# antonilo/unsupervised_detection

Hardware: NVIDIA H100
Metric: frame-pairs/sec adversarial train step 256x448 (higher is better)
Workload: dtype bf16

## Files before the change

### include/cis_b200.h

```cpp
#ifndef CIS_B200_H_
#define CIS_B200_H_
#include <stdint.h>
#include <stddef.h>

#ifdef __cplusplus
extern "C" {
#endif

typedef void* cis_stream_t;

enum { CIS_OK = 0, CIS_ERR_BAD_ARG = 1, CIS_ERR_UNSUPPORTED = 2, CIS_ERR_CUDA = 3 };
enum { CIS_ACT_NONE = 0, CIS_ACT_ELU = 1, CIS_ACT_LEAKY = 2 };
enum { CIS_MAX_TAPS = 49, CIS_MAX_SRC = 4 };

typedef struct {
  const void* ptr;
  int32_t pitch;
  int32_t c_off;
  int32_t chunks;
  int32_t n_mod;
} CisSrc;

typedef struct {
  int32_t N, H, W;
// ... 58 lines not shown
  int32_t Cout;
  int32_t K_pad;
  int32_t splits;
  int32_t tma;
  int32_t nh;
  int32_t nwg;
} CisWgrad;

const char* cis_last_error(void);
int cis_version(void);
uint32_t cis_crc32c(uint32_t crc, const void* data, size_t n);
int cis_host_resize_bilinear_legacy(const float* src, int32_t H, int32_t W, int32_t C, float* dst, int32_t OH, int32_t OW);
int cis_host_bgr8_to_rgb_resized(const unsigned char* bgr, int32_t H, int32_t W, float* dst, int32_t OH, int32_t OW);

int cis_conv_igemm(const CisConv* d, cis_stream_t stream);
int cis_set_persist_mode(int mode);
int cis_conv_wgrad(const CisWgrad* d, cis_stream_t stream);

int cis_pack_weights(const float* w, const int32_t* kmap, int32_t K_pad, int32_t rows, int32_t cout, int32_t sn, const int32_t* nmap,
                     void* wp, cis_stream_t stream);
int cis_pack_weights_tiled(const float* w, const int32_t* kmap, int32_t cin8, int32_t ntaps, int32_t n_tiles, int32_t BN, int32_t cout,
                           int32_t sn, const int32_t* nmap, void* out, int32_t thin, cis_stream_t stream);
int cis_unpack_wgrad(const float* dwp, const int32_t* kmap, int32_t K_pad, int32_t cout, int32_t nsplit, float* dw, const float* colpart,
                     int32_t nblocks, int32_t nch, float* db, int32_t layout, cis_stream_t stream);
int cis_bn_fold(const float* w, const float* bias, const float* gamma, const float* beta, int64_t nw, int32_t cout, float* w_eff,
                float* b_eff, cis_stream_t stream);
int cis_bn_chain(const float* w, const float* bias, const float* gamma, float* dw_eff_to_dw, const float* db_eff, int64_t nw,
                 int32_t cout, float* dbias, float* dgamma, float* dbeta, cis_stream_t stream);

enum { CIS_JOB_PACK = 0, CIS_JOB_PACK_TILED = 1, CIS_JOB_UNPACK = 2, CIS_JOB_BN_FOLD = 3, CIS_JOB_BN_CHAIN = 4 };
// ... 124 lines not shown
```

### unsupervised_detection_b200/_lib.py

```python
import ctypes as C
import os

_HERE = os.path.dirname(os.path.abspath(__file__))
LIB_PATH = os.path.join(_HERE, os.environ.get('CIS_LIB_NAME', 'libcis_b200.so'))

MAX_TAPS, MAX_SRC = 49, 4
ACT_NONE, ACT_ELU, ACT_LEAKY = 0, 1, 2
RESIZE_BILINEAR, RESIZE_NEAREST = 0, 1


class CisSrc(C.Structure):
    _fields_ = [('ptr', C.c_void_p), ('pitch', C.c_int32), ('c_off', C.c_int32), ('chunks', C.c_int32), ('n_mod', C.c_int32)]


class CisParamJob(C.Structure):
    _fields_ = [('kind', C.c_int32), ('i', C.c_int32 * 8), ('n', C.c_int64), ('p', C.c_void_p * 8)]


JOB_PACK, JOB_PACK_TILED, JOB_UNPACK, JOB_BN_FOLD, JOB_BN_CHAIN = range(5)


class CisSub(C.Structure):
    _fields_ = [('tap0', C.c_int32), ('ntaps', C.c_int32), ('hoy', C.c_int32), ('hox', C.c_int32), ('OH', C.c_int32), ('OW', C.c_int32),
                ('oa', C.c_int32), ('ob', C.c_int32), ('wpack', C.c_void_p)]
# ... 81 lines not shown
    'cis_cast_bf16_to_f32': [_p, _i64, _i32, _i32, _i32, _p],
    'cis_cast_bf16_to_f32_scaled': [_p, _i64, _i32, _i32, _i32, _f32, _p],
    'cis_charbonnier_bwd': [_p, _p, _p, _i32, _i64, _i32, _i32, _f32, _p, _p, _p, _p],
    'cis_dense_image_warp_bwd': [_p, _i32, _i32, _p, _f32, _i32, _i32, _i32, _i32, _p, _p, _p, _p],
    'cis_cost_volume_bwd': [_p, _i32, _i32, _p, _i32, _i32, _p, _i32, _i32, _i32, _i32, _p, _p, _p],
    'cis_resize_f32_bwd_to_bf16_scaled': [_p, _i32, _i32, _i32, _i32, _i32, _i32, _p, _i32, _f32],
    'cis_warp_costvol_bwd': [_p, _i32, _i32, _p, _i32, _i32, _p, _f32, _i32, _i32, _i32, _i32, _p, _i32, _i32, _p, _i32, _i32, _p, _i32, _i32,
                             _p, _i32, _i32, _i32, _p, _p, _p],
    'cis_parity_split_bf16': [_p, _i32, _i32, _i32, _i32, _i32, _i32, _p, _i32],
    'cis_warp_costvol_r': [_p, _i32, _i32, _p, _i32, _i32, _p, _f32, _i32, _i32, _i32, _i32, _p, _i32, _i32, _i32],
    'cis_cost_volume_bwd_r': [_p, _i32, _i32, _p, _i32, _i32, _p, _i32, _i32, _i32, _i32, _p, _p, _p, _i32],
    'cis_warp_costvol_bwd_r': [_p, _i32, _i32, _p, _i32, _i32, _p, _f32, _i32, _i32, _i32, _i32, _p, _i32, _i32, _p, _i32, _i32, _p, _i32, _i32,
                               _p, _i32, _i32, _i32, _p, _p, _p, _i32],
}
EXPORTS = sorted(list(_PROTOS) + ['cis_last_error', 'cis_version', 'cis_set_persist_mode', 'cis_crc32c', 'cis_host_resize_bilinear_legacy',
                                  'cis_host_bgr8_to_rgb_resized'])

_lib = None


def load():
    global _lib
    if _lib is None:
        if not os.path.exists(LIB_PATH):
            raise RuntimeError('libcis_b200.so not built: run `python -c "import __graft_entry__ as g; g.build()"` '
                               '(no CPU fallback exists for the product path)')
        lib = C.CDLL(LIB_PATH)
        lib.cis_last_error.restype = C.c_char_p
        lib.cis_version.restype = C.c_int
        lib.cis_set_persist_mode.argtypes = [C.c_int]
        lib.cis_set_persist_mode.restype = C.c_int
        lib.cis_crc32c.argtypes = [C.c_uint32, C.c_void_p, C.c_size_t]
        lib.cis_crc32c.restype = C.c_uint32
        lib.cis_host_resize_bilinear_legacy.argtypes = [C.c_void_p, C.c_int32, C.c_int32, C.c_int32, C.c_void_p, C.c_int32, C.c_int32]
        lib.cis_host_resize_bilinear_legacy.restype = C.c_int
        lib.cis_host_bgr8_to_rgb_resized.argtypes = [C.c_void_p, C.c_int32, C.c_int32, C.c_void_p, C.c_int32, C.c_int32]
        lib.cis_host_bgr8_to_rgb_resized.restype = C.c_int
        for name, args in _PROTOS.items():
            fn = getattr(lib, name)
            fn.argtypes = list(args) + [C.c_void_p]
            fn.restype = C.c_int
        _lib = lib
    return _lib


def check(rc, what=''):
    if rc != 0:
        raise RuntimeError('libcis_b200 %s failed (code %d): %s' % (what, rc, load().cis_last_error().decode()))


def call(name, *args):
    check(getattr(load(), name)(*args), name)
# ... 1 lines not shown
```

### unsupervised_detection_b200/csrc/conv_igemm.cu

```cuda
#include "ptx.cuh"
#include "../../include/cis_b200.h"
#include "common.cuh"
#include <cuda.h>
#include <stdlib.h>
#include <string.h>


namespace cis {

#ifdef CIS_TRACE
__device__ unsigned long long* g_trace = nullptr;
__device__ int g_trace_cap = 0;
#define CIS_TRACE_AT(slot)                                                                                         \
  do {                                                                                                             \
    if (g_trace && blockIdx.x == 0 && blockIdx.y == 0 && blockIdx.z == 0 && (slot) < g_trace_cap) g_trace[(slot)] = clock64(); \
  } while (0)
#else
#define CIS_TRACE_AT(slot) ((void)0)
#endif

static constexpr int kBM = 128;
static constexpr int kBK = 64;
static constexpr int kAStage = kBM * 128;
static constexpr int kThreads = 256;
// ... 471 lines not shown
        const int t = g / p.OW;
        const int oh = t % p.OH;
        const int n = t / p.OH;
        return (size_t)(n * p.DH + oh * p.osh + p.oa) * p.DW + ow * p.osw + p.ob;
      });
    }
    cluster_sync_all();
  }
  if (tid == 0) CIS_TRACE_AT(3);
}


static constexpr int kHaloMaxBStages = 8;
struct HaloMaps {
  CUtensorMap m[CIS_MAX_SRC * 4];
};

template <int NK, int MT, int BN, int MTM>
__device__ __forceinline__ void halo_issue_stage(float (&acc)[MTM][BN], const uint32_t hlo, uint32_t blo, const uint32_t* s_aoff, const int gt,
                                                 const uint32_t ahi, const uint32_t bhi, const uint32_t a_mstep, const uint32_t a_half,
                                                 const uint32_t bstep, const bool first) {
  uint32_t off0 = s_aoff[0], off1 = gt > 1 ? s_aoff[1] : 0u;
  int tt = 0;
#pragma unroll 1
  do {
    const uint32_t off2 = tt + 2 < gt ? s_aoff[tt + 2] : 0u;
    const uint32_t alo = hlo + off0;
    const uint32_t acc0 = (uint32_t)(!(first && tt == 0));
    wg_fence();
#pragma unroll
    for (int m = 0; m < MT; ++m) {
// ... 21 lines not shown
                                               const uint32_t a_half, const uint32_t bstep, const bool first) {
  static_assert(MTM >= 1 && MTM <= 4, "1..4 stacked tiles");
  if (MT == 1) halo_issue_nk<1>(nk16, acc, hlo, blo, s_aoff, gt, ahi, bhi, a_mstep, a_half, bstep, first);
  else if constexpr (MTM >= 2) {
    if (MT == 2) halo_issue_nk<2>(nk16, acc, hlo, blo, s_aoff, gt, ahi, bhi, a_mstep, a_half, bstep, first);
    else if constexpr (MTM >= 3) {
      if (MT == 3) halo_issue_nk<3>(nk16, acc, hlo, blo, s_aoff, gt, ahi, bhi, a_mstep, a_half, bstep, first);
      else if constexpr (MTM >= 4) halo_issue_nk<4>(nk16, acc, hlo, blo, s_aoff, gt, ahi, bhi, a_mstep, a_half, bstep, first);
    }
  }
  wg_wait<0>();
}

__host__ __device__ __forceinline__ int thin_plane_bytes(int HP) { return (HP * 16 + 127) & ~127; }
__host__ __device__ __forceinline__ int halo_nsteps(int thin, int ntaps) { return thin == 8 ? (ntaps + 1) / 2 : ntaps; }
__device__ __forceinline__ uint32_t halo_step_off(const CisConv& p, const int t0, const int nt, const int s, const int Wh, const uint32_t plane16) {
  if (!p.thin) return (uint32_t)((p.dh[t0 + s] * Wh + p.dw[t0 + s]) * 8);
  const int ta = p.thin == 8 ? 2 * s : s;
  const uint32_t o0 = (uint32_t)(p.dh[t0 + ta] * Wh + p.dw[t0 + ta]);
  if (p.thin == 16) return o0 | (plane16 << 16);
  const uint32_t o1 = ta + 1 < nt ? (uint32_t)(p.dh[t0 + ta + 1] * Wh + p.dw[t0 + ta + 1]) : o0;
  return o0 | ((o1 - o0) << 16);
}

template <int BN, int NWG>
__global__ void __launch_bounds__(HaloCfg<BN, NWG>::kThreads, 1) conv_halo_kernel(const __grid_constant__ CisConv p, const int halo_stage_bytes, const int BS, const int NHS,
                                                        const __grid_constant__ HaloMaps maps, const int use_tma, const int G) {
  using Cfg = HaloCfg<BN, NWG>;
  constexpr int kBStage = BN * 128;
  constexpr int kHMmaWarp_ = Cfg::kMmaWarp, kHThreads_ = Cfg::kThreads;
  extern __shared__ uint8_t smem_raw[];
  __shared__ uint64_t bars[2 * 2 + 2 * kHaloMaxBStages + 1];
  __shared__ uint32_t s_aoff[CIS_MAX_TAPS];
  __shared__ SrcS s_src[CIS_MAX_SRC];

  const int tid = threadIdx.x, warp = tid >> 5, lane = tid & 31;
  const int MT = p.MT, MTC = NWG * MT, d = p.dil;
  const int nph = p.nph > 1 ? p.nph : 1;
  const int Wh = 8 + p.ex, Hh = 16 * MTC + p.ey, HP = Wh * Hh;
  const int thin = p.thin;
  const uint32_t wstep = thin ? BN * 32 : kBStage;
  const uint32_t stage_bytes = (uint32_t)G * wstep;
  const uint32_t tile_base = (smem_u32(smem_raw) + 1023u) & ~1023u;
  const uint32_t h_base = tile_base;
  const uint32_t b_base = tile_base + NHS * halo_stage_bytes;
  int* pixtab = reinterpret_cast<int*>(smem_raw + (b_base + BS * stage_bytes - smem_u32(smem_raw)));
  const uint32_t bar_hfull = smem_u32(&bars[0]), bar_hempty = smem_u32(&bars[2]);
  const uint32_t bar_bfull = smem_u32(&bars[4]), bar_bempty = smem_u32(&bars[4 + kHaloMaxBStages]);
  const uint32_t bar_accum = smem_u32(&bars[4 + 2 * kHaloMaxBStages]);

  const bool grouped = p.nsub > 1;
  const int tap0 = grouped ? p.sub[blockIdx.z].tap0 : 0, ntaps = grouped ? p.sub[blockIdx.z].ntaps : p.ntaps;
  const int nst = halo_nsteps(thin, ntaps);
  const int hoy = grouped ? p.sub[blockIdx.z].hoy : p.hoy, hox = grouped ? p.sub[blockIdx.z].hox : p.hox;
  const int OHs = grouped ? p.sub[blockIdx.z].OH : p.OH, OWs = grouped ? p.sub[blockIdx.z].OW : p.OW;
// ... 44 lines not shown
    }
    mbar_init(bar_accum, 128 * NWG);
    fence_mbar_init();
  }
  if (use_tma && tid < p.nsrc) tma_prefetch_desc(&maps.m[tid]);
  pdl_wait();
  if (tid < BN) s_bias[tid] = p.bias ? p.bias[ny * BN + tid] : 0.f;
  __syncthreads();
  if (tid == 0) CIS_TRACE_AT(0);

  if (warp < kHMmaWarp_) {
   if (warp < 4) {
    if (use_tma) {
      if (tid == 0) {
        int hcount = 0;
        for (int vc = 0; vc < nchunks * nph; ++vc) {
          const int cc = vc / nph, ph = vc - cc * nph;
          if (nph > 1 && p.ph_tap[ph + 1] == p.ph_tap[ph]) continue;
          const int hs = hcount % NHS;
          mbar_wait(bar_hempty + 8 * hs, (uint32_t)(((hcount / NHS) & 1) ^ 1));
          ++hcount;
          int c = (cc_lo + cc) * 8, si = 0;
          while (si < p.nsrc - 1 && c >= s_src[si].chunks) {
            c -= s_src[si].chunks;
            ++si;
          }
          const int nmod = s_src[si].n_mod;
          if (thin) {
            const int npl = thin / 8, pb16 = thin_plane_bytes(HP);
            mbar_expect_tx(bar_hfull + 8 * hs, (uint32_t)(npl * HP * 16));
            for (int q = 0; q < npl; ++q) {
              int cq = q, sq = 0;
              while (sq < p.nsrc - 1 && cq >= s_src[sq].chunks) {
                cq -= s_src[sq].chunks;
                ++sq;
              }
              const int nm = s_src[sq].n_mod;
              tma_load_4d(h_base + hs * halo_stage_bytes + q * pb16, &maps.m[sq], bar_hfull + 8 * hs, cq * 8, tx * 8 + hox, ty * 16 * MTC + hoy,
                          nm ? (n % nm) : n);
            }
            continue;
          }
          mbar_expect_tx(bar_hfull + 8 * hs, (uint32_t)(HP * 128));
          tma_load_4d(h_base + hs * halo_stage_bytes, &maps.m[si * nph + ph], bar_hfull + 8 * hs, c * 8, pb + d * (tx * 8 + hox),
                      pa + d * (ty * 16 * MTC + hoy), nmod ? (n % nmod) : n);
        }
      }
      __syncwarp();
    } else if (warp != 2) {
      const int hid = warp == 3 ? tid - 32 : tid;
      const int j = hid & 7, pl = hid >> 3;
      for (int cc = 0; cc < nchunks; ++cc) {
        const int hs = cc % NHS;
        mbar_wait(bar_hempty + 8 * hs, (uint32_t)(((cc / NHS) & 1) ^ 1));
        const int rem = m_chunks - (cc_lo + cc) * 8;
// ... 31 lines not shown
          cp_async_wait<1>();
          fence_proxy_async();
          mbar_arrive(bar_hfull + 8 * ((cc - 1) % NHS));
        }
      }
      if (NHS > 1) {
        cp_async_wait<0>();
        fence_proxy_async();
        mbar_arrive(bar_hfull + 8 * ((nchunks - 1) % NHS));
      }
    }
    if (tid == 64) {
      const uint8_t* wt = reinterpret_cast<const uint8_t*>(wpack) + ((size_t)ny * nchunks_all + cc_lo) * nst * wstep;
      int bs = 0;
      uint32_t bph = 1;
      for (int vc = 0; vc < nchunks * nph; ++vc) {
        const int cc = vc / nph, ph = vc - cc * nph;
        const int tlo = nph > 1 ? p.ph_tap[ph] : 0, thi = nph > 1 ? p.ph_tap[ph + 1] : nst;
        for (int t0 = tlo; t0 < thi; t0 += G) {
          const uint32_t bytes = (uint32_t)min(G, thi - t0) * wstep;
          mbar_wait(bar_bempty + 8 * bs, bph);
          mbar_expect_tx(bar_bfull + 8 * bs, bytes);
          bulk_g2s(b_base + bs * stage_bytes, wt + (size_t)(cc * nst + t0) * wstep, bytes, bar_bfull + 8 * bs);
          if (++bs == BS) {
            bs = 0;
            bph ^= 1u;
          }
        }
      }
    }
    __syncwarp();
   }

  } else {
    const int wg = NWG > 1 ? (warp - kHMmaWarp_) >> 2 : 0;
    const int wtid = tid - (kHMmaWarp_ + 4 * wg) * 32;
    constexpr int MTM = Cfg::kMaxMT;
    float acc[MTM][BN];
    const uint32_t pix = thin ? 16u : 128u;
    const uint32_t ahi = thin ? desc_hi_ns((uint32_t)Wh * pix) : desc_hi((uint32_t)Wh * pix), bhi = thin ? desc_hi_ns(256) : desc_hi(1024);
    const uint32_t a_mstep = (16u * Wh * pix) >> 4;
    const uint32_t a_half = (8u * Wh * pix) >> 4;
    const uint32_t a_wg = (uint32_t)(wg * MT) * a_mstep;
    int bs = 0, hs = 0, it = 0;
    uint32_t bph = 0, hph = 0;
    bool any = false;
    for (int vc = 0; vc < nchunks * nph; ++vc) {
      const int cc = vc / nph, ph = vc - cc * nph;
      const int tlo = nph > 1 ? p.ph_tap[ph] : 0, thi = nph > 1 ? p.ph_tap[ph + 1] : nst;
      if (thi == tlo) continue;
      const int rem = m_chunks - (cc_lo + cc) * 8;
      const int nk16 = rem >= 8 ? 4 : (rem + 1) / 2;
      mbar_wait(bar_hfull + 8 * hs, hph);
      if (vc == 0 && wtid == 0 && wg == 0) CIS_TRACE_AT(1);
      const uint32_t hlo = desc_lo(h_base + hs * halo_stage_bytes, thin ? 0 : 16) + a_wg;
      for (int t0 = tlo; t0 < thi; t0 += G, ++it) {
        const int gt = min(G, thi - t0);
        mbar_wait(bar_bfull + 8 * bs, bph);
        if (wtid == 0 && wg == 0) CIS_TRACE_AT(8 + 2 * it);
        const uint32_t blo = desc_lo(b_base + bs * stage_bytes, thin ? 128 : 16);
        halo_issue_any<BN, MTM>(nk16, acc, hlo, blo, s_aoff + t0, gt, MT, ahi, bhi, a_mstep, a_half, wstep >> 4, !any);
        if (wtid == 0) {
          mbar_arrive(bar_bempty + 8 * bs);
          if (t0 + G >= thi) mbar_arrive(bar_hempty + 8 * hs);
          if (wg == 0) CIS_TRACE_AT(9 + 2 * it);
        }
        any = true;
        if (++bs == BS) {
          bs = 0;
          bph ^= 1u;
        }
      }
      if (++hs == NHS) {
        hs = 0;
        hph ^= 1u;
// ... 193 lines not shown
        int z, tx, ty, n;
        decode(w, z, tx, ty, n);
        const int hox = grouped ? p.sub[z].hox : p.hox, hoy = grouped ? p.sub[z].hoy : p.hoy;
        for (int cc = 0; cc < nchunks; ++cc) {
          mbar_wait(bar_hempty + 8 * hs, hph);
          int c = cc * 8, si = 0;
          while (si < p.nsrc - 1 && c >= p.src[si].chunks) {
            c -= p.src[si].chunks;
            ++si;
          }
          int nmod = p.src[0].n_mod;
          if (si == 1) nmod = p.src[1].n_mod;
          if (si == 2) nmod = p.src[2].n_mod;
          if (si == 3) nmod = p.src[3].n_mod;
          if (thin) {
            const int npl = thin / 8, pb16 = thin_plane_bytes(HP);
            mbar_expect_tx(bar_hfull + 8 * hs, (uint32_t)(npl * HP * 16));
            for (int q = 0; q < npl; ++q) {
              int cq = q, sq = 0;
              while (sq < p.nsrc - 1 && cq >= p.src[sq].chunks) {
                cq -= p.src[sq].chunks;
                ++sq;
              }
              const int nm = p.src[sq].n_mod;
              tma_load_4d(h_base + hs * halo_stage_bytes + q * pb16, &maps.m[sq], bar_hfull + 8 * hs, cq * 8, tx * 8 + hox, ty * 16 * MT + hoy,
                          nm ? (n % nm) : n);
            }
          } else {
            mbar_expect_tx(bar_hfull + 8 * hs, (uint32_t)(HP * 128));
            tma_load_4d(h_base + hs * halo_stage_bytes, &maps.m[si], bar_hfull + 8 * hs, c * 8, tx * 8 + hox, ty * 16 * MT + hoy,
                        nmod ? (n % nmod) : n);
          }
          if (++hs == NHS) {
            hs = 0;
            hph ^= 1u;
          }
        }
      }
    }
  } else if (warp == 13) {
    if (lane == 0) {
      const uint8_t* wt = reinterpret_cast<const uint8_t*>(p.wpack);
      const int nst = s_sbase[1];
      if (ws) {
        if ((int)blockIdx.x < total) {
          mbar_expect_tx(bar_bfull, (uint32_t)(nchunks * s_sbase[nsb] * wstep));
          for (int z = 0; z < nsb; ++z) {
            const uint8_t* wz = grouped ? reinterpret_cast<const uint8_t*>(p.sub[z].wpack) : wt;
            const int per = nchunks * (s_sbase[z + 1] - s_sbase[z]);
            for (int it = 0; it < per; it += 8) {
              const int nt = min(8, per - it);
              bulk_g2s(b_base + (s_sbase[z] + it) * wstep, wz + (size_t)it * wstep, (uint32_t)(nt * wstep), bar_bfull);
            }
          }
        }
      } else {
        int bs = 0;
        uint32_t bph = 1;
        for (int w = blockIdx.x; w < total; w += gridDim.x) {
          for (int cc = 0; cc < nchunks; ++cc) {
            for (int t0 = 0; t0 < nst; t0 += G) {
              const uint32_t bytes = (uint32_t)min(G, nst - t0) * wstep;
              mbar_wait(bar_bempty + 8 * bs, bph);
              mbar_expect_tx(bar_bfull + 8 * bs, bytes);
              bulk_g2s(b_base + bs * stage_bytes, wt + (size_t)(cc * nst + t0) * wstep, bytes, bar_bfull + 8 * bs);
              if (++bs == BS) {
                bs = 0;
                bph ^= 1u;
              }
            }
          }
        }
      }
    }
  } else if (warp < 4) {
    const int wtid = tid;
    constexpr int MTM = (kPMaxAccCols / BN) < 4 ? kPMaxAccCols / BN : 4;
    float acc[MTM][BN];
    const uint32_t pix = thin ? 16u : 128u;
    const uint32_t ahi = thin ? desc_hi_ns((uint32_t)Wh * pix) : desc_hi((uint32_t)Wh * pix), bhi = thin ? desc_hi_ns(256) : desc_hi(1024);
    const uint32_t a_mstep = (16u * Wh * pix) >> 4;
    const uint32_t a_half = (8u * Wh * pix) >> 4;
    int hs = 0, bs = 0, as = 0;
    uint32_t hph = 0, bph = 0, tph = 1;
    if (ws && (int)blockIdx.x < total) mbar_wait(bar_bfull, 0u);
    int wi = 0;
    for (int w = blockIdx.x; w < total; w += gridDim.x, ++wi) {
      if (wtid == 0) CIS_TRACE_AT(8 + 5 * wi);
      int z, tx, ty, n;
      decode(w, z, tx, ty, n);
      const int nst = s_sbase[z + 1] - s_sbase[z];
      const uint32_t* so = s_aoff + s_sbase[z];
      for (int cc = 0; cc < nchunks; ++cc) {
        const int rem = m_chunks - cc * 8;
        const int nk16 = rem >= 8 ? 4 : (rem + 1) / 2;
        mbar_wait(bar_hfull + 8 * hs, hph);
        if (cc == 0 && wtid == 0) CIS_TRACE_AT(10 + 5 * wi);
        const uint32_t hlo = desc_lo(h_base + hs * halo_stage_bytes, thin ? 0 : 16);
        const int gstep = ws ? nst : G;
        for (int t0 = 0; t0 < nst; t0 += gstep) {
          const int gt = min(gstep, nst - t0);
          if (!ws) mbar_wait(bar_bfull + 8 * bs, bph);
          const uint32_t blo = desc_lo(ws ? b_base + (uint32_t)(s_sbase[z] + cc * nst) * wstep : b_base + bs * stage_bytes, thin ? 128 : 16);
          halo_issue_any<BN, MTM>(nk16, acc, hlo, blo, so + t0, gt, MT, ahi, bhi, a_mstep, a_half, wstep >> 4, (cc | t0) == 0);
          if (wtid == 0) {
            if (!ws) mbar_arrive(bar_bempty + 8 * bs);
            if (t0 + gstep >= nst) mbar_arrive(bar_hempty + 8 * hs);
          }
          if (!ws && ++bs == BS) {
            bs = 0;
            bph ^= 1u;
          }
        }
        if (++hs == NHS) {
          hs = 0;
          hph ^= 1u;
        }
      }
// ... 527 lines not shown
#ifdef CIS_TRACE
extern "C" int cis_trace_set(unsigned long long* buf, int cap) {
  cudaError_t e = cudaMemcpyToSymbol(cis::g_trace, &buf, sizeof(buf));
  if (e == cudaSuccess) e = cudaMemcpyToSymbol(cis::g_trace_cap, &cap, sizeof(cap));
  return e == cudaSuccess ? CIS_OK : cis_set_cuda_error(e, "cis_trace_set");
}
#endif

static int g_persist_mode = -1;
extern "C" int cis_set_persist_mode(int mode) {
  g_persist_mode = mode;
  return CIS_OK;
}

template <int BN, int NWG>
static int launch_halo(const CisConv* d, cudaStream_t st) {
  const int MTC = d->MT * NWG;
  const int Wh = 8 + d->ex, Hh = 16 * MTC + d->ey, HP = Wh * Hh;
  const int thin = d->thin;
  const int halo_stage = ((thin ? thin / 8 * thin_plane_bytes(HP) : HP * 128) + 1023) & ~1023;
  int chunks = 0;
  for (int i = 0; i < d->nsrc; ++i) chunks += d->src[i].chunks;
  if (thin && ((thin != 8 && thin != 16) || chunks * 8 != thin || d->dil != 1 || d->nph > 1))
    return cis_set_error(CIS_ERR_BAD_ARG, "cis_conv_igemm(halo): the compact format needs 8 or 16 undilated input channels");
  const int nchunks = (chunks + 7) / 8;
  const int nsub = d->nsub > 1 ? d->nsub : 1;
  const int nsp = (nsub == 1 && d->splits > 1) ? d->splits : 1;
  const int cper = (nchunks + nsp - 1) / nsp;
  const int nhs = cper > 1 ? 2 : 1;
  const int dd = d->dil;
  int tiles = 0, ntaps_max = d->ntaps;
  if (nsub > 1) {
    if (nsub > 4 || dd != 1 || d->splits > 1 || d->nph > 1) return cis_set_error(CIS_ERR_BAD_ARG, "cis_conv_igemm(halo): bad grouped launch");
    ntaps_max = 0;
    int tsum = 0;
    for (int i = 0; i < nsub; ++i) {
      const int t = ((d->sub[i].OW + 7) / 8) * ((d->sub[i].OH + 16 * MTC - 1) / (16 * MTC));
      if (t > tiles) tiles = t;
      if (d->sub[i].ntaps > ntaps_max) ntaps_max = d->sub[i].ntaps;
      if (d->sub[i].ntaps < 1 || d->sub[i].tap0 != tsum || !d->sub[i].wpack) return cis_set_error(CIS_ERR_BAD_ARG, "cis_conv_igemm(halo): bad sub-problem");
      tsum += d->sub[i].ntaps;
    }
    if (tsum != d->ntaps) return cis_set_error(CIS_ERR_BAD_ARG, "cis_conv_igemm(halo): sub-problem taps must add up to ntaps");
  } else {
    const int Hp0 = (d->OH + dd - 1) / dd, Wp0 = (d->OW + dd - 1) / dd;
    tiles = ((Wp0 + 7) / 8) * ((Hp0 + 16 * MTC - 1) / (16 * MTC));
  }
  if (thin == 8) {
    for (int i = 0; i < nsub; ++i) {
      const int t0 = nsub > 1 ? d->sub[i].tap0 : 0, nt = nsub > 1 ? d->sub[i].ntaps : d->ntaps;
      for (int t = t0 + 1; t < t0 + nt; ++t)
        if (d->dh[t] * (8 + d->ex) + d->dw[t] < d->dh[t - 1] * (8 + d->ex) + d->dw[t - 1])
          return cis_set_error(CIS_ERR_BAD_ARG, "cis_conv_igemm(halo): compact 8-channel taps must be listed in increasing halo offset");
    }
  }
  const int nst_max = halo_nsteps(thin, ntaps_max);
  const long ncta_all = (long)tiles * dd * dd * d->N * d->n_tiles * nsp * nsub;
  static const int g_env = getenv("CIS_HALO_G") ? atoi(getenv("CIS_HALO_G")) : 0;
  static const int stage_kb = getenv("CIS_HALO_STAGE_KB") ? atoi(getenv("CIS_HALO_STAGE_KB")) : 48;
  const int kB = thin ? BN * 32 : BN * 128;
  int G = g_env > 0 ? g_env : (stage_kb * 1024) / kB;
  if (G < 1) G = 1;
  if (G > nst_max) G = nst_max;
  const int fixed = nhs * halo_stage + HP * 4 + 1024;
  static const int lim_small_kb = getenv("CIS_HALO_SMALL_KB") ? atoi(getenv("CIS_HALO_SMALL_KB")) : 226;
  static const int lim_kb_wide = getenv("CIS_HALO_LIMIT_KB") ? atoi(getenv("CIS_HALO_LIMIT_KB")) : 113;
  static const int lim_kb_thin = getenv("CIS_HALO_LIMIT_THIN_KB") ? atoi(getenv("CIS_HALO_LIMIT_THIN_KB")) : 113;
// ... 13 lines not shown
  static int attr_smem = 0;
  if (smem > attr_smem) {
    cudaError_t e = cudaFuncSetAttribute(conv_halo_kernel<BN, NWG>, cudaFuncAttributeMaxDynamicSharedMemorySize, smem);
    if (e != cudaSuccess) return cis_set_cuda_error(e, "cudaFuncSetAttribute(conv_halo)");
    attr_smem = smem;
  }

  int splits = d->splits > 1 ? d->splits : 1;
  if (splits > 1) {
    const int per = (nchunks + splits - 1) / splits;
    if ((!d->sk_scratch && !d->sk_cluster) || d->sk_counters || (splits - 1) * per >= nchunks || (d->sk_cluster && splits > 8))
      return cis_set_error(CIS_ERR_BAD_ARG, "cis_conv_igemm(halo): bad split-K setup");
  }
  dim3 grid(tiles * dd * dd * d->N, d->n_tiles, nsub > 1 ? nsub : splits);
  HaloMaps maps;
  const int nph = d->nph > 1 ? d->nph : 1;
  static const int dil_tma = getenv("CIS_DIL_TMA") ? atoi(getenv("CIS_DIL_TMA")) : 1;
  int use_tma = ((d->dil == 1 || dil_tma) && Wh * d->dil <= 256 && Hh * d->dil <= 256) ? 1 : 0;
  for (int i = 0; use_tma && !thin && i < d->nsrc - 1; ++i)
    if (d->src[i].chunks % 8) use_tma = 0;
  for (int i = 0; use_tma && i < d->nsrc; ++i) {
    if (((uintptr_t)d->src[i].ptr + (size_t)d->src[i].c_off * 2) % 16) use_tma = 0;
    for (int ph = 0; use_tma && ph < nph; ++ph)
      if (!(thin ? encode_src_map(&maps.m[i], d->src[i], d->N, d->H, d->W, Wh, Hh, 1, 0, 0, 1, 8, CU_TENSOR_MAP_SWIZZLE_NONE)
                 : encode_src_map(&maps.m[i * nph + ph], d->src[i], d->N, d->H, d->W, Wh, Hh, nph > 1 ? 2 : 1, ph >> 1, ph & 1, d->dil)))
        use_tma = 0;
  }
  if (!use_tma) memset(&maps, 0, sizeof(maps));
  if (thin && !use_tma) return cis_set_error(CIS_ERR_UNSUPPORTED, "cis_conv_igemm(halo): the compact format needs the TMA halo path");
  if (nph > 1 && !use_tma) return cis_set_error(CIS_ERR_UNSUPPORTED, "cis_conv_igemm(halo): stride-2 phases need the TMA halo path");
  const int persist_mode = g_persist_mode >= 0 ? g_persist_mode : (getenv("CIS_PERSIST_MODE") ? atoi(getenv("CIS_PERSIST_MODE")) : 1);
  static const int p_min_tiles = getenv("CIS_PERSIST_MIN_TILES") ? atoi(getenv("CIS_PERSIST_MIN_TILES")) : 296;
  static const int p_ws_kb = getenv("CIS_PERSIST_WS_KB") ? atoi(getenv("CIS_PERSIST_WS_KB")) : 112;
  if constexpr (BN <= kPMaxAccCols && NWG == 1) {
   if (persist_mode > 0 && use_tma && d->n_tiles == 1 && splits == 1 && nph == 1 && (nsub == 1 || nchunks == 1) && dd == 1 &&
       d->MT * BN <= kPMaxAccCols) {
    int total = tiles * d->N, per_tile = nchunks * nst_max;
    if (nsub > 1) {
      total = per_tile = 0;
      for (int i = 0; i < nsub; ++i) {
        total += ((d->sub[i].OW + 7) / 8) * ((d->sub[i].OH + 16 * d->MT - 1) / (16 * d->MT)) * d->N;
        per_tile += halo_nsteps(thin, d->sub[i].ntaps);
      }
    }
    const int acc_stage = d->MT * BN * (int)kAccColBytes;
    const int AS = 2;
    const int fixed_p = AS * acc_stage + 1024;
    const int ws_bytes = per_tile * kB;
    int p_nhs = nchunks >= 3 ? 4 : 3;
    while (p_nhs > 2 && p_nhs * halo_stage + fixed_p + (ws_bytes <= p_ws_kb * 1024 ? ws_bytes : 2 * G * kB) > 226 * 1024) --p_nhs;
// ... 27 lines not shown
    }
   }
  }
  cudaError_t le = (splits > 1 && d->sk_cluster)
                       ? launch_pdl_zcluster(conv_halo_kernel<BN, NWG>, grid, dim3(HaloCfg<BN, NWG>::kThreads), smem, st, splits, *d, halo_stage, BS, nhs, maps,
                                             use_tma, G)
                       : launch_pdl(conv_halo_kernel<BN, NWG>, grid, dim3(HaloCfg<BN, NWG>::kThreads), smem, st, *d, halo_stage, BS, nhs, maps, use_tma, G);
  if (le != cudaSuccess) return cis_set_cuda_error(le, "launch(conv_halo)");
  if (splits > 1 && !d->sk_cluster) {
    le = launch_splitk_finish<BN>(d, grid, st);
    if (le != cudaSuccess) return cis_set_cuda_error(le, "launch(splitk_finish)");
  }
  return cis_check_launch("conv_halo");
}

extern "C" int cis_conv_igemm(const CisConv* d, cis_stream_t stream) {
  if (!d || d->ntaps < 1 || d->ntaps > CIS_MAX_TAPS || d->nsrc < 1 || d->nsrc > CIS_MAX_SRC || d->K_pad % 64 != 0 || d->K_pad <= 0 ||
      d->n_tiles < 1 || !d->wpack)
    return cis_set_error(CIS_ERR_BAD_ARG, "cis_conv_igemm: bad descriptor");
  int chunks = 0;
  for (int i = 0; i < d->nsrc; ++i) {
    if ((d->src[i].pitch | d->src[i].c_off) & 7) return cis_set_error(CIS_ERR_BAD_ARG, "cis_conv_igemm: source pitch/c_off must be multiples of 8");
    chunks += d->src[i].chunks;
  }
  if (d->ntaps * chunks * 8 > d->K_pad) return cis_set_error(CIS_ERR_BAD_ARG, "cis_conv_igemm: K_pad smaller than taps*channels");
  if (d->mode == 1 && !d->outf) return cis_set_error(CIS_ERR_BAD_ARG, "cis_conv_igemm: mode 1 needs outf");
  if ((d->add_pre || d->add_post) && (((d->add_pre_pitch | d->add_pre_coff | d->add_post_pitch | d->add_post_coff | d->out_ch) & 7) != 0))
    return cis_set_error(CIS_ERR_BAD_ARG, "cis_conv_igemm: residual slices must be 8-channel aligned");
  cudaStream_t st = (cudaStream_t)stream;
  if (d->halo) {
    if (d->MT < 1 || d->MT > 4 || d->MT * d->BN > kMaxAccCols || d->nwg < 0 || d->nwg > 2 || (d->nwg == 2 && d->BN < 64) || d->dil < 1 ||
        d->sh != 1 || d->sw != 1 || d->ey < 0 || d->ex < 0 ||
        (d->dil > 1 && (d->OH != d->H || d->OW != d->W)) || (d->nph > 1 && (d->nph != 4 || d->dil != 1 || d->ph_tap[0] != 0 || d->ph_tap[4] != d->ntaps)))
      return cis_set_error(CIS_ERR_BAD_ARG, "cis_conv_igemm(halo): bad tile parameters");
    switch (d->BN) {
      case 16: return launch_halo<16, 1>(d, st);
      case 32: return launch_halo<32, 1>(d, st);
      case 64: return d->nwg == 2 ? launch_halo<64, 2>(d, st) : launch_halo<64, 1>(d, st);
      case 128: return d->nwg == 2 ? launch_halo<128, 2>(d, st) : launch_halo<128, 1>(d, st);
      default: return cis_set_error(CIS_ERR_UNSUPPORTED, "cis_conv_igemm: BN must be 16/32/64/128");
    }
  }
  switch (d->BN) {
    case 16: return launch_fwd<16>(d, st);
    case 32: return launch_fwd<32>(d, st);
    case 64: return launch_fwd<64>(d, st);
    case 128: return launch_fwd<128>(d, st);
    default: return cis_set_error(CIS_ERR_UNSUPPORTED, "cis_conv_igemm: BN must be 16/32/64/128");
  }
}

template <int NH, int NWG>
static int launch_wgrad_halo_t(const CisWgrad* d, cudaStream_t st, int nch64, int Wh, int Hh, int hoy, int hox, int halo_bytes) {
  using Cfg = WgradHaloCfg<NH>;
  const bool wg_halves = NWG == 2 && d->Cout > 64;
// ... 98 lines not shown
```

Before: 639.3.

## Route thin stride-2 convs through phase-split halo kernel with row-pack weight TMA

Stride-2 convolutions with 8 or 16 input channels, which used to run on the generic implicit-GEMM path, are now rewritten as four parity-phase stride-1 halo convolutions. The halo tile is loaded per phase through TMA and the weights come from a 2D tensor map that indexes the original packed rows, so no repack is needed. A host cost model chooses the MT tile height, and the new path is taken only when the plan would launch at least 296 CTAs. The aim is to replace per-tap gathers with smem halo reuse; the costs are larger halo stages, extra TMA descriptors and more complex control flow.

```diff
diff --git a/include/cis_b200.h b/include/cis_b200.h
--- a/include/cis_b200.h
+++ b/include/cis_b200.h
@@ -96,6 +96,7 @@
 int cis_host_bgr8_to_rgb_resized(const unsigned char* bgr, int32_t H, int32_t W, float* dst, int32_t OH, int32_t OW);
 
 int cis_conv_igemm(const CisConv* d, cis_stream_t stream);
+int cis_conv_s2_phase_plan(const CisConv* d, CisConv* h, int16_t* wk);
 int cis_set_persist_mode(int mode);
 int cis_conv_wgrad(const CisWgrad* d, cis_stream_t stream);
 
diff --git a/unsupervised_detection_b200/_lib.py b/unsupervised_detection_b200/_lib.py
--- a/unsupervised_detection_b200/_lib.py
+++ b/unsupervised_detection_b200/_lib.py
@@ -119,7 +119,7 @@
                                _p, _i32, _i32, _i32, _p, _p, _p, _i32],
 }
 EXPORTS = sorted(list(_PROTOS) + ['cis_last_error', 'cis_version', 'cis_set_persist_mode', 'cis_crc32c', 'cis_host_resize_bilinear_legacy',
-                                  'cis_host_bgr8_to_rgb_resized'])
+                                  'cis_host_bgr8_to_rgb_resized', 'cis_conv_s2_phase_plan'])
 
 _lib = None
 
@@ -141,6 +141,8 @@
         lib.cis_host_resize_bilinear_legacy.restype = C.c_int
         lib.cis_host_bgr8_to_rgb_resized.argtypes = [C.c_void_p, C.c_int32, C.c_int32, C.c_void_p, C.c_int32, C.c_int32]
         lib.cis_host_bgr8_to_rgb_resized.restype = C.c_int
+        lib.cis_conv_s2_phase_plan.argtypes = [C.POINTER(CisConv), C.POINTER(CisConv), C.POINTER(C.c_int16)]
+        lib.cis_conv_s2_phase_plan.restype = C.c_int
         for name, args in _PROTOS.items():
             fn = getattr(lib, name)
             fn.argtypes = list(args) + [C.c_void_p]
diff --git a/unsupervised_detection_b200/csrc/conv_igemm.cu b/unsupervised_detection_b200/csrc/conv_igemm.cu
--- a/unsupervised_detection_b200/csrc/conv_igemm.cu
+++ b/unsupervised_detection_b200/csrc/conv_igemm.cu
@@ -509,7 +509,15 @@
 static constexpr int kHaloMaxBStages = 8;
 struct HaloMaps {
   CUtensorMap m[CIS_MAX_SRC * 4];
+  CUtensorMap w;
+  int wrow;
+  int16_t wk[2 * CIS_MAX_TAPS];
 };
+__device__ __forceinline__ void wrow_load(const HaloMaps& maps, const uint32_t dst, const uint32_t bar, const int s0, const int ns, const int n0,
+                                          const int BN) {
+  for (int s = 0; s < ns; ++s)
+    for (int j = 0; j < 2; ++j) tma_load_2d(dst + (uint32_t)(s * BN * 32 + j * BN * 16), &maps.w, bar, maps.wk[2 * (s0 + s) + j], n0);
+}
 
 template <int NK, int MT, int BN, int MTM>
 __device__ __forceinline__ void halo_issue_stage(float (&acc)[MTM][BN], const uint32_t hlo, uint32_t blo, const uint32_t* s_aoff, const int gt,
@@ -561,13 +569,39 @@
 
 __host__ __device__ __forceinline__ int thin_plane_bytes(int HP) { return (HP * 16 + 127) & ~127; }
 __host__ __device__ __forceinline__ int halo_nsteps(int thin, int ntaps) { return thin == 8 ? (ntaps + 1) / 2 : ntaps; }
+__device__ __forceinline__ uint32_t halo_tap_off(const CisConv& p, const int t, const int Wh, const uint32_t plane16) {
+  int ph = 0;
+  if (p.nph > 1)
+    while (ph < p.nph - 1 && t >= p.ph_tap[ph + 1]) ++ph;
+  return (uint32_t)(ph * (p.thin / 8)) * plane16 + (uint32_t)(p.dh[t] * Wh + p.dw[t]);
+}
 __device__ __forceinline__ uint32_t halo_step_off(const CisConv& p, const int t0, const int nt, const int s, const int Wh, const uint32_t plane16) {
   if (!p.thin) return (uint32_t)((p.dh[t0 + s] * Wh + p.dw[t0 + s]) * 8);
   const int ta = p.thin == 8 ? 2 * s : s;
-  const uint32_t o0 = (uint32_t)(p.dh[t0 + ta] * Wh + p.dw[t0 + ta]);
+  const uint32_t o0 = halo_tap_off(p, t0 + ta, Wh, plane16);
   if (p.thin == 16) return o0 | (plane16 << 16);
-  const uint32_t o1 = ta + 1 < nt ? (uint32_t)(p.dh[t0 + ta + 1] * Wh + p.dw[t0 + ta + 1]) : o0;
+  const uint32_t o1 = ta + 1 < nt ? halo_tap_off(p, t0 + ta + 1, Wh, plane16) : o0;
   return o0 | ((o1 - o0) << 16);
+}
+template <typename Src>
+__device__ __forceinline__ void thin_halo_load(const CisConv& p, const Src* src, const HaloMaps& maps, const uint32_t dst, const uint32_t bar,
+                                               const int HP, const int x0, const int y0, const int n) {
+  const int nph = p.nph > 1 ? p.nph : 1, npl = p.thin / 8, pb16 = thin_plane_bytes(HP);
+  int nld = 0;
+  for (int ph = 0; ph < nph; ++ph) nld += nph == 1 || p.ph_tap[ph + 1] > p.ph_tap[ph];
+  mbar_expect_tx(bar, (uint32_t)(nld * npl * HP * 16));
+  for (int ph = 0; ph < nph; ++ph) {
+    if (nph > 1 && p.ph_tap[ph + 1] == p.ph_tap[ph]) continue;
+    for (int q = 0; q < npl; ++q) {
+      int cq = q, sq = 0;
+      while (sq < p.nsrc - 1 && cq >= src[sq].chunks) {
+        cq -= src[sq].chunks;
+        ++sq;
+      }
+      const int nm = src[sq].n_mod;
+      tma_load_4d(dst + (ph * npl + q) * pb16, &maps.m[sq * nph + ph], bar, cq * 8, x0, y0, nm ? (n % nm) : n);
+    }
+  }
 }
 
 template <int BN, int NWG>
@@ -586,6 +620,7 @@
   const int nph = p.nph > 1 ? p.nph : 1;
   const int Wh = 8 + p.ex, Hh = 16 * MTC + p.ey, HP = Wh * Hh;
   const int thin = p.thin;
+  const int nhph = thin ? 1 : nph;
   const uint32_t wstep = thin ? BN * 32 : kBStage;
   const uint32_t stage_bytes = (uint32_t)G * wstep;
   const uint32_t tile_base = (smem_u32(smem_raw) + 1023u) & ~1023u;
@@ -660,9 +695,9 @@
     if (use_tma) {
       if (tid == 0) {
         int hcount = 0;
-        for (int vc = 0; vc < nchunks * nph; ++vc) {
-          const int cc = vc / nph, ph = vc - cc * nph;
-          if (nph > 1 && p.ph_tap[ph + 1] == p.ph_tap[ph]) continue;
+        for (int vc = 0; vc < nchunks * nhph; ++vc) {
+          const int cc = vc / nhph, ph = vc - cc * nhph;
+          if (nhph > 1 && p.ph_tap[ph + 1] == p.ph_tap[ph]) continue;
           const int hs = hcount % NHS;
           mbar_wait(bar_hempty + 8 * hs, (uint32_t)(((hcount / NHS) & 1) ^ 1));
           ++hcount;
@@ -673,18 +708,7 @@
           }
           const int nmod = s_src[si].n_mod;
           if (thin) {
-            const int npl = thin / 8, pb16 = thin_plane_bytes(HP);
-            mbar_expect_tx(bar_hfull + 8 * hs, (uint32_t)(npl * HP * 16));
-            for (int q = 0; q < npl; ++q) {
-              int cq = q, sq = 0;
-              while (sq < p.nsrc - 1 && cq >= s_src[sq].chunks) {
-                cq -= s_src[sq].chunks;
-                ++sq;
-              }
-              const int nm = s_src[sq].n_mod;
-              tma_load_4d(h_base + hs * halo_stage_bytes + q * pb16, &maps.m[sq], bar_hfull + 8 * hs, cq * 8, tx * 8 + hox, ty * 16 * MTC + hoy,
-                          nm ? (n % nm) : n);
-            }
+            thin_halo_load(p, s_src, maps, h_base + hs * halo_stage_bytes, bar_hfull + 8 * hs, HP, tx * 8 + hox, ty * 16 * MTC + hoy, n);
             continue;
           }
           mbar_expect_tx(bar_hfull + 8 * hs, (uint32_t)(HP * 128));
@@ -746,14 +770,15 @@
       const uint8_t* wt = reinterpret_cast<const uint8_t*>(wpack) + ((size_t)ny * nchunks_all + cc_lo) * nst * wstep;
       int bs = 0;
       uint32_t bph = 1;
-      for (int vc = 0; vc < nchunks * nph; ++vc) {
-        const int cc = vc / nph, ph = vc - cc * nph;
-        const int tlo = nph > 1 ? p.ph_tap[ph] : 0, thi = nph > 1 ? p.ph_tap[ph + 1] : nst;
+      for (int vc = 0; vc < nchunks * nhph; ++vc) {
+        const int cc = vc / nhph, ph = vc - cc * nhph;
+        const int tlo = nhph > 1 ? p.ph_tap[ph] : 0, thi = nhph > 1 ? p.ph_tap[ph + 1] : nst;
         for (int t0 = tlo; t0 < thi; t0 += G) {
           const uint32_t bytes = (uint32_t)min(G, thi - t0) * wstep;
           mbar_wait(bar_bempty + 8 * bs, bph);
           mbar_expect_tx(bar_bfull + 8 * bs, bytes);
-          bulk_g2s(b_base + bs * stage_bytes, wt + (size_t)(cc * nst + t0) * wstep, bytes, bar_bfull + 8 * bs);
+          if (maps.wrow) wrow_load(maps, b_base + bs * stage_bytes, bar_bfull + 8 * bs, t0, min(G, thi - t0), ny * BN, BN);
+          else bulk_g2s(b_base + bs * stage_bytes, wt + (size_t)(cc * nst + t0) * wstep, bytes, bar_bfull + 8 * bs);
           if (++bs == BS) {
             bs = 0;
             bph ^= 1u;
@@ -770,16 +795,17 @@
     constexpr int MTM = Cfg::kMaxMT;
     float acc[MTM][BN];
     const uint32_t pix = thin ? 16u : 128u;
-    const uint32_t ahi = thin ? desc_hi_ns((uint32_t)Wh * pix) : desc_hi((uint32_t)Wh * pix), bhi = thin ? desc_hi_ns(256) : desc_hi(1024);
+    const uint32_t ahi = thin ? desc_hi_ns((uint32_t)Wh * pix) : desc_hi((uint32_t)Wh * pix);
+    const uint32_t bhi = thin ? desc_hi_ns(maps.wrow ? 128u : 256u) : desc_hi(1024), b_lbo = maps.wrow ? BN * 16u : thin ? 128u : 16u;
     const uint32_t a_mstep = (16u * Wh * pix) >> 4;
     const uint32_t a_half = (8u * Wh * pix) >> 4;
     const uint32_t a_wg = (uint32_t)(wg * MT) * a_mstep;
     int bs = 0, hs = 0, it = 0;
     uint32_t bph = 0, hph = 0;
     bool any = false;
-    for (int vc = 0; vc < nchunks * nph; ++vc) {
-      const int cc = vc / nph, ph = vc - cc * nph;
-      const int tlo = nph > 1 ? p.ph_tap[ph] : 0, thi = nph > 1 ? p.ph_tap[ph + 1] : nst;
+    for (int vc = 0; vc < nchunks * nhph; ++vc) {
+      const int cc = vc / nhph, ph = vc - cc * nhph;
+      const int tlo = nhph > 1 ? p.ph_tap[ph] : 0, thi = nhph > 1 ? p.ph_tap[ph + 1] : nst;
       if (thi == tlo) continue;
       const int rem = m_chunks - (cc_lo + cc) * 8;
       const int nk16 = rem >= 8 ? 4 : (rem + 1) / 2;
@@ -790,7 +816,7 @@
         const int gt = min(G, thi - t0);
         mbar_wait(bar_bfull + 8 * bs, bph);
         if (wtid == 0 && wg == 0) CIS_TRACE_AT(8 + 2 * it);
-        const uint32_t blo = desc_lo(b_base + bs * stage_bytes, thin ? 128 : 16);
+        const uint32_t blo = desc_lo(b_base + bs * stage_bytes, b_lbo);
         halo_issue_any<BN, MTM>(nk16, acc, hlo, blo, s_aoff + t0, gt, MT, ahi, bhi, a_mstep, a_half, wstep >> 4, !any);
         if (wtid == 0) {
           mbar_arrive(bar_bempty + 8 * bs);
@@ -1014,18 +1040,7 @@
           if (si == 2) nmod = p.src[2].n_mod;
           if (si == 3) nmod = p.src[3].n_mod;
           if (thin) {
-            const int npl = thin / 8, pb16 = thin_plane_bytes(HP);
-            mbar_expect_tx(bar_hfull + 8 * hs, (uint32_t)(npl * HP * 16));
-            for (int q = 0; q < npl; ++q) {
-              int cq = q, sq = 0;
-              while (sq < p.nsrc - 1 && cq >= p.src[sq].chunks) {
-                cq -= p.src[sq].chunks;
-                ++sq;
-              }
-              const int nm = p.src[sq].n_mod;
-              tma_load_4d(h_base + hs * halo_stage_bytes + q * pb16, &maps.m[sq], bar_hfull + 8 * hs, cq * 8, tx * 8 + hox, ty * 16 * MT + hoy,
-                          nm ? (n % nm) : n);
-            }
+            thin_halo_load(p, p.src, maps, h_base + hs * halo_stage_bytes, bar_hfull + 8 * hs, HP, tx * 8 + hox, ty * 16 * MT + hoy, n);
           } else {
             mbar_expect_tx(bar_hfull + 8 * hs, (uint32_t)(HP * 128));
             tma_load_4d(h_base + hs * halo_stage_bytes, &maps.m[si], bar_hfull + 8 * hs, c * 8, tx * 8 + hox, ty * 16 * MT + hoy,
@@ -1045,7 +1060,8 @@
       if (ws) {
         if ((int)blockIdx.x < total) {
           mbar_expect_tx(bar_bfull, (uint32_t)(nchunks * s_sbase[nsb] * wstep));
-          for (int z = 0; z < nsb; ++z) {
+          if (maps.wrow) wrow_load(maps, b_base, bar_bfull, 0, nst, 0, BN);
+          for (int z = 0; z < nsb && !maps.wrow; ++z) {
             const uint8_t* wz = grouped ? reinterpret_cast<const uint8_t*>(p.sub[z].wpack) : wt;
             const int per = nchunks * (s_sbase[z + 1] - s_sbase[z]);
             for (int it = 0; it < per; it += 8) {
@@ -1063,7 +1079,8 @@
               const uint32_t bytes = (uint32_t)min(G, nst - t0) * wstep;
               mbar_wait(bar_bempty + 8 * bs, bph);
               mbar_expect_tx(bar_bfull + 8 * bs, bytes);
-              bulk_g2s(b_base + bs * stage_bytes, wt + (size_t)(cc * nst + t0) * wstep, bytes, bar_bfull + 8 * bs);
+              if (maps.wrow) wrow_load(maps, b_base + bs * stage_bytes, bar_bfull + 8 * bs, t0, min(G, nst - t0), 0, BN);
+              else bulk_g2s(b_base + bs * stage_bytes, wt + (size_t)(cc * nst + t0) * wstep, bytes, bar_bfull + 8 * bs);
               if (++bs == BS) {
                 bs = 0;
                 bph ^= 1u;
@@ -1078,7 +1095,8 @@
     constexpr int MTM = (kPMaxAccCols / BN) < 4 ? kPMaxAccCols / BN : 4;
     float acc[MTM][BN];
     const uint32_t pix = thin ? 16u : 128u;
-    const uint32_t ahi = thin ? desc_hi_ns((uint32_t)Wh * pix) : desc_hi((uint32_t)Wh * pix), bhi = thin ? desc_hi_ns(256) : desc_hi(1024);
+    const uint32_t ahi = thin ? desc_hi_ns((uint32_t)Wh * pix) : desc_hi((uint32_t)Wh * pix);
+    const uint32_t bhi = thin ? desc_hi_ns(maps.wrow ? 128u : 256u) : desc_hi(1024), b_lbo = maps.wrow ? BN * 16u : thin ? 128u : 16u;
     const uint32_t a_mstep = (16u * Wh * pix) >> 4;
     const uint32_t a_half = (8u * Wh * pix) >> 4;
     int hs = 0, bs = 0, as = 0;
@@ -1101,7 +1119,7 @@
         for (int t0 = 0; t0 < nst; t0 += gstep) {
           const int gt = min(gstep, nst - t0);
           if (!ws) mbar_wait(bar_bfull + 8 * bs, bph);
-          const uint32_t blo = desc_lo(ws ? b_base + (uint32_t)(s_sbase[z] + cc * nst) * wstep : b_base + bs * stage_bytes, thin ? 128 : 16);
+          const uint32_t blo = desc_lo(ws ? b_base + (uint32_t)(s_sbase[z] + cc * nst) * wstep : b_base + bs * stage_bytes, b_lbo);
           halo_issue_any<BN, MTM>(nk16, acc, hlo, blo, so + t0, gt, MT, ahi, bhi, a_mstep, a_half, wstep >> 4, (cc | t0) == 0);
           if (wtid == 0) {
             if (!ws) mbar_arrive(bar_bempty + 8 * bs);
@@ -1659,14 +1677,15 @@
 }
 
 template <int BN, int NWG>
-static int launch_halo(const CisConv* d, cudaStream_t st) {
+static int launch_halo(const CisConv* d, cudaStream_t st, const int16_t* wk = nullptr) {
   const int MTC = d->MT * NWG;
   const int Wh = 8 + d->ex, Hh = 16 * MTC + d->ey, HP = Wh * Hh;
   const int thin = d->thin;
-  const int halo_stage = ((thin ? thin / 8 * thin_plane_bytes(HP) : HP * 128) + 1023) & ~1023;
+  const int nph = d->nph > 1 ? d->nph : 1;
+  const int halo_stage = ((thin ? nph * (thin / 8) * thin_plane_bytes(HP) : HP * 128) + 1023) & ~1023;
   int chunks = 0;
   for (int i = 0; i < d->nsrc; ++i) chunks += d->src[i].chunks;
-  if (thin && ((thin != 8 && thin != 16) || chunks * 8 != thin || d->dil != 1 || d->nph > 1))
+  if (thin && ((thin != 8 && thin != 16) || chunks * 8 != thin || d->dil != 1))
     return cis_set_error(CIS_ERR_BAD_ARG, "cis_conv_igemm(halo): the compact format needs 8 or 16 undilated input channels");
   const int nchunks = (chunks + 7) / 8;
   const int nsub = d->nsub > 1 ? d->nsub : 1;
@@ -1695,7 +1714,8 @@
     for (int i = 0; i < nsub; ++i) {
       const int t0 = nsub > 1 ? d->sub[i].tap0 : 0, nt = nsub > 1 ? d->sub[i].ntaps : d->ntaps;
       for (int t = t0 + 1; t < t0 + nt; ++t)
-        if (d->dh[t] * (8 + d->ex) + d->dw[t] < d->dh[t - 1] * (8 + d->ex) + d->dw[t - 1])
+        if (!(nph > 1 && (t == d->ph_tap[1] || t == d->ph_tap[2] || t == d->ph_tap[3])) &&
+            d->dh[t] * (8 + d->ex) + d->dw[t] < d->dh[t - 1] * (8 + d->ex) + d->dw[t - 1])
           return cis_set_error(CIS_ERR_BAD_ARG, "cis_conv_igemm(halo): compact 8-channel taps must be listed in increasing halo offset");
     }
   }
@@ -1739,7 +1759,6 @@
   }
   dim3 grid(tiles * dd * dd * d->N, d->n_tiles, nsub > 1 ? nsub : splits);
   HaloMaps maps;
-  const int nph = d->nph > 1 ? d->nph : 1;
   static const int dil_tma = getenv("CIS_DIL_TMA") ? atoi(getenv("CIS_DIL_TMA")) : 1;
   int use_tma = ((d->dil == 1 || dil_tma) && Wh * d->dil <= 256 && Hh * d->dil <= 256) ? 1 : 0;
   for (int i = 0; use_tma && !thin && i < d->nsrc - 1; ++i)
@@ -1747,18 +1766,31 @@
   for (int i = 0; use_tma && i < d->nsrc; ++i) {
     if (((uintptr_t)d->src[i].ptr + (size_t)d->src[i].c_off * 2) % 16) use_tma = 0;
     for (int ph = 0; use_tma && ph < nph; ++ph)
-      if (!(thin ? encode_src_map(&maps.m[i], d->src[i], d->N, d->H, d->W, Wh, Hh, 1, 0, 0, 1, 8, CU_TENSOR_MAP_SWIZZLE_NONE)
+      if (!(thin ? encode_src_map(&maps.m[i * nph + ph], d->src[i], d->N, d->H, d->W, Wh, Hh, nph > 1 ? 2 : 1, ph >> 1, ph & 1, 1, 8,
+                                  CU_TENSOR_MAP_SWIZZLE_NONE)
                  : encode_src_map(&maps.m[i * nph + ph], d->src[i], d->N, d->H, d->W, Wh, Hh, nph > 1 ? 2 : 1, ph >> 1, ph & 1, d->dil)))
         use_tma = 0;
   }
   if (!use_tma) memset(&maps, 0, sizeof(maps));
   if (thin && !use_tma) return cis_set_error(CIS_ERR_UNSUPPORTED, "cis_conv_igemm(halo): the compact format needs the TMA halo path");
   if (nph > 1 && !use_tma) return cis_set_error(CIS_ERR_UNSUPPORTED, "cis_conv_igemm(halo): stride-2 phases need the TMA halo path");
+  maps.wrow = 0;
+  if (wk) {
+    EncodeTiledFn enc = get_encode_tiled();
+    const cuuint64_t dims[2] = {(cuuint64_t)d->K_pad, (cuuint64_t)d->n_tiles * BN}, strides[1] = {(cuuint64_t)d->K_pad * 2};
+    const cuuint32_t box[2] = {8, (cuuint32_t)BN}, es[2] = {1, 1};
+    if (!thin || nsub > 1 || !enc ||
+        enc(&maps.w, CU_TENSOR_MAP_DATA_TYPE_BFLOAT16, 2, const_cast<void*>(d->wpack), dims, strides, box, es, CU_TENSOR_MAP_INTERLEAVE_NONE,
+            CU_TENSOR_MAP_SWIZZLE_NONE, CU_TENSOR_MAP_L2_PROMOTION_L2_128B, CU_TENSOR_MAP_FLOAT_OOB_FILL_NONE) != CUDA_SUCCESS)
+      return cis_set_error(CIS_ERR_UNSUPPORTED, "cis_conv_igemm(halo): row-pack weight map");
+    maps.wrow = 1;
+    memcpy(maps.wk, wk, sizeof(maps.wk));
+  }
   const int persist_mode = g_persist_mode >= 0 ? g_persist_mode : (getenv("CIS_PERSIST_MODE") ? atoi(getenv("CIS_PERSIST_MODE")) : 1);
   static const int p_min_tiles = getenv("CIS_PERSIST_MIN_TILES") ? atoi(getenv("CIS_PERSIST_MIN_TILES")) : 296;
   static const int p_ws_kb = getenv("CIS_PERSIST_WS_KB") ? atoi(getenv("CIS_PERSIST_WS_KB")) : 112;
   if constexpr (BN <= kPMaxAccCols && NWG == 1) {
-   if (persist_mode > 0 && use_tma && d->n_tiles == 1 && splits == 1 && nph == 1 && (nsub == 1 || nchunks == 1) && dd == 1 &&
+   if (persist_mode > 0 && use_tma && d->n_tiles == 1 && splits == 1 && (nph == 1 || thin) && (nsub == 1 || nchunks == 1) && dd == 1 &&
        d->MT * BN <= kPMaxAccCols) {
     int total = tiles * d->N, per_tile = nchunks * nst_max;
     if (nsub > 1) {
@@ -1816,6 +1848,81 @@
   return cis_check_launch("conv_halo");
 }
 
+static bool s2_phase_plan(const CisConv* g, CisConv* h, int16_t* wk) {
+  int chunks = 0;
+  for (int i = 0; i < g->nsrc; ++i) {
+    chunks += g->src[i].chunks;
+    if (((uintptr_t)g->src[i].ptr + (size_t)g->src[i].c_off * 2) % 16) return false;
+  }
+  const int thin = chunks * 8, BN = g->BN;
+  if (g->sh != 2 || g->sw != 2 || (thin != 8 && thin != 16) || g->splits > 1 || g->nsub > 1 || g->nph > 1 || g->dil > 1 || g->H < 2 ||
+      g->W < 2 || BN > 128 || g->K_pad > 32767)
+    return false;
+  const int nt = g->ntaps;
+  int order[CIS_MAX_TAPS], bounds[5] = {0, 0, 0, 0, 0}, k = 0;
+  for (int q = 0; q < 4; ++q) {
+    for (int t = 0; t < nt; ++t)
+      if (((g->dh[t] & 1) << 1 | (g->dw[t] & 1)) == q) order[k++] = t;
+    bounds[q + 1] = k;
+  }
+  int hoy = 1 << 20, hox = 1 << 20, ey = 0, ex = 0;
+  for (int t = 0; t < nt; ++t) {
+    hoy = min(hoy, g->dh[t] >> 1);
+    hox = min(hox, g->dw[t] >> 1);
+  }
+  *h = *g;
+  for (int i = 0; i < nt; ++i) {
+    h->dh[i] = (int16_t)((g->dh[order[i]] >> 1) - hoy);
+    h->dw[i] = (int16_t)((g->dw[order[i]] >> 1) - hox);
+    ey = max(ey, (int)h->dh[i]);
+    ex = max(ex, (int)h->dw[i]);
+  }
+  const int nst = halo_nsteps(thin, nt), kb = BN * 32, tiles_x = (g->OW + 7) / 8, nsm = cis_num_sms();
+  int best_mt = 0;
+  double best = 0.0;
+  for (int MT = 1; MT <= 4; ++MT) {
+    if (MT * BN > kMaxAccCols || 8 + ex > 256 || 16 * MT + ey > 256) continue;
+    const int HP = (8 + ex) * (16 * MT + ey);
+    const int halo = (4 * (thin / 8) * thin_plane_bytes(HP) + 1023) & ~1023, smem = halo + HP * 4 + 2048 + 2 * kb;
+    if (smem > 227 * 1024) continue;
+    const int tiles_y = (g->OH + 16 * MT - 1) / (16 * MT);
+    if ((double)g->OH * g->OW < 0.2 * tiles_y * 16 * MT * tiles_x * 8) continue;
+    const long ncta = (long)g->N * tiles_x * tiles_y * g->n_tiles;
+    const int cps = max(1, min(225 * 1024 / smem, 4));
+    const double t_mma = MT * 2.0 * BN * nst * 0.25, t_mem = (double)kb * nst / 40.0 + halo / 40.0;
+    const double t_cta = fmax(t_mma, t_mem) + (4000.0 + 1500.0 * MT) / cps;
+    const double cost = (double)((ncta + (long)nsm * cps - 1) / ((long)nsm * cps)) * cps * t_cta / fmin((double)cps, fmax(1.0, (double)ncta / nsm));
+    if (!best_mt || cost < best - 1e-9) {
+      best = cost;
+      best_mt = MT;
+    }
+  }
+  if (!best_mt || (long)g->N * tiles_x * ((g->OH + 16 * best_mt - 1) / (16 * best_mt)) * g->n_tiles < 296) return false;
+  h->halo = 1;
+  h->sh = h->sw = 1;
+  h->dil = 1;
+  h->MT = best_mt;
+  h->nwg = 1;
+  h->hoy = hoy;
+  h->hox = hox;
+  h->ey = ey;
+  h->ex = ex;
+  h->nph = 4;
+  for (int q = 0; q < 5; ++q) h->ph_tap[q] = bounds[q];
+  h->thin = thin;
+  h->splits = 0;
+  h->sk_cluster = 0;
+  for (int s = 0; s < nst; ++s)
+    for (int j = 0; j < 2; ++j) {
+      const int i = thin == 8 ? 2 * s + j : s;
+      wk[2 * s + j] = (int16_t)(thin == 8 ? (i < nt ? order[i] * 8 : g->K_pad) : order[i] * 16 + 8 * j);
+    }
+  return true;
+}
+extern "C" int cis_conv_s2_phase_plan(const CisConv* d, CisConv* h, int16_t* wk) {
+  return d && h && wk && !d->halo && s2_phase_plan(d, h, wk) ? 1 : 0;
+}
+
 extern "C" int cis_conv_igemm(const CisConv* d, cis_stream_t stream) {
   if (!d || d->ntaps < 1 || d->ntaps > CIS_MAX_TAPS || d->nsrc < 1 || d->nsrc > CIS_MAX_SRC || d->K_pad % 64 != 0 || d->K_pad <= 0 ||
       d->n_tiles < 1 || !d->wpack)
@@ -1841,6 +1948,16 @@
       case 64: return d->nwg == 2 ? launch_halo<64, 2>(d, st) : launch_halo<64, 1>(d, st);
       case 128: return d->nwg == 2 ? launch_halo<128, 2>(d, st) : launch_halo<128, 1>(d, st);
       default: return cis_set_error(CIS_ERR_UNSUPPORTED, "cis_conv_igemm: BN must be 16/32/64/128");
+    }
+  }
+  CisConv h;
+  int16_t wk[2 * CIS_MAX_TAPS];
+  if (s2_phase_plan(d, &h, wk)) {
+    switch (h.BN) {
+      case 16: return launch_halo<16, 1>(&h, st, wk);
+      case 32: return launch_halo<32, 1>(&h, st, wk);
+      case 64: return launch_halo<64, 1>(&h, st, wk);
+      case 128: return launch_halo<128, 1>(&h, st, wk);
     }
   }
   switch (d->BN) {
```

Measured after the change: 660.8, median of 6. 1.03x the previous value.
